# stgl/scarplet

Hardware: AMD Instinct MI355X
Metric: Mpixel·template/s (DEM pixels × ages × orientations / s) (higher is better)
Workload: dtype f32

## Files before the change

scarplet_amd/csrc/sc_fft.hip:

```cpp
#include "sc_internal.h"
#include <math.h>
#include <type_traits>
#include <string.h>

struct TileDev {
    int i0, j0, vy, vx, gi0, gj0;
};

#ifndef SC_I1_XLANE
#define SC_I1_XLANE 1
#endif
#ifndef SC_I2_RD1
#define SC_I2_RD1 1
#endif
#ifndef SC_LDS_WR1
#define SC_LDS_WR1 0
#endif
#ifndef SC_LDS_RD1
#define SC_LDS_RD1 1
#endif
#ifndef SC_H2_XLANE
#define SC_H2_XLANE 1
#endif
#ifndef SC_F1C_HOLD
// ... 593 lines not shown
                                              : make_float2(va[u], vb[u]);
        }
        lds_barrier();
        if (!SC_DBGBIT(dbg, 2)) fft4_lines<TX, false, true>(sm, twr);
#if SC_F1C_HOLD
        if (step + 1 < 2 * RBW && (!MIX || ((step + 1) & 1) == 0)) fetch(rb0 + ((step + 1) >> 1));
#else
        if (step + 1 < 2 * RBW) fetch(rb0 + ((step + 1) >> 1));
#endif
        float2* out = blk + (size_t)(pair * 2 + pl) * plane + (size_t)rb * 4 * TX;
        if (!SC_DBGBIT(dbg, 4))
#pragma unroll 4
        for (int e = 2 * tid; e < 4 * TX; e += 2 * NT) {
            int cb = e >> 4, rr = (e >> 2) & 3, cc = e & 3;
            float2 x0 = sm[lidx<TX>(rr, 4 * cb + cc)], x1 = sm[lidx<TX>(rr, 4 * cb + cc + 1)];
            *reinterpret_cast<float4*>(out + e) = make_float4(x0.x, x0.y, x1.x, x1.y);
        }
        lds_barrier();
    }
}

__global__ void __launch_bounds__(64)
k_tile_norms(const double* __restrict__ part, int nrb, double* __restrict__ norms) {
    const double2* p = reinterpret_cast<const double2*>(part) + (size_t)blockIdx.x * nrb;
    double s2 = 0.0, s4 = 0.0;
    for (int i = threadIdx.x; i < nrb; i += 64) {
        const double2 v = p[i];
        s2 += v.x;
        s4 += v.y;
    }
    for (int sft = 32; sft > 0; sft >>= 1) {
        s2 += __shfl_down(s2, sft, 64);
        s4 += __shfl_down(s4, sft, 64);
    }
    if (threadIdx.x == 0) {
        norms[2 * blockIdx.x] = s2;
        norms[2 * blockIdx.x + 1] = s4;
    }
}

__device__ __forceinline__ bool templ_rowblock_used(const TemplDev& t, int rb, int Ty) {
    bool any = false;
#pragma unroll
    for (int rr = 0; rr < 4; ++rr) {
        int r = 4 * rb + rr;
        int p = (r <= t.pmax) ? r : r - Ty;
        any |= p >= t.pmin && p <= t.pmax;
    }
    return any;
}

template <int TX>
__global__ void __launch_bounds__(fft_threads(TX), fft_waves(TX))
k_fwd_rows_templ(const TemplDev* __restrict__ templ, int first,
                 const float* __restrict__ win_w,
                 const uint8_t* __restrict__ win_m,
                 const double* __restrict__ sums, int Ty,
                 const float2* __restrict__ tw, float2* __restrict__ blk) {
    extern __shared__ __attribute__((aligned(16))) float2 sm[];
    FftTw<TX> twr;
    twr.load(tw);
    constexpr int NT = fft_threads(TX);
    const int rb = blockIdx.x;
    const TemplDev t = templ[first + blockIdx.y];
    const float alpha = sc_fft_alpha(sums, first + blockIdx.y);
    const size_t plane = (size_t)Ty * TX;
    float2* out = blk + (size_t)blockIdx.y * plane + (size_t)rb * 4 * TX;
    bool any = false;
    int prow[4];
#pragma unroll
    for (int rr = 0; rr < 4; ++rr) {
        int r = 4 * rb + rr;
        int p = (r <= t.pmax) ? r : r - Ty;
        prow[rr] = (p >= t.pmin && p <= t.pmax) ? p : INT_MIN;
        any |= prow[rr] != INT_MIN;
    }
    if (!any) return;
    {
        constexpr int NF = 4 * TX / NT;
        float w[NF];
        uint8_t m[NF];
#pragma unroll
        for (int u = 0; u < NF; ++u) {
            const int e = threadIdx.x + u * NT;
            const int rr = e / TX, s = e - rr * TX;
            const int q = (s <= t.qmax) ? s : s - TX;
            w[u] = 0.f;
            m[u] = 0;
            if (prow[rr] != INT_MIN && q >= t.qmin && q <= t.qmax) {
                size_t o = (size_t)t.win_off + (size_t)(prow[rr] - t.pmin) * t.ww + (q - t.qmin);
                w[u] = win_w[o];
                m[u] = win_m[o];
            }
        }
#pragma unroll
        for (int u = 0; u < NF; ++u) {
            const int e = threadIdx.x + u * NT;
            const int rr = e / TX, s = e - rr * TX;
            sm[lidx<TX>(rr, s)] = make_float2(alpha * w[u], m[u] ? 1.f : 0.f);
        }
    }
    lds_barrier();
    fft4_lines<TX, false>(sm, twr);
#pragma unroll 4
    for (int e = 2 * threadIdx.x; e < 4 * TX; e += 2 * NT) {
        int cb = e >> 4, rr = (e >> 2) & 3, cc = e & 3;
        float2 x0 = sm[lidx<TX>(rr, 4 * cb + cc)], x1 = sm[lidx<TX>(rr, 4 * cb + cc + 1)];
        *reinterpret_cast<float4*>(out + e) = make_float4(x0.x, x0.y, x1.x, x1.y);
    }
}

template <int TY>
__global__ void __launch_bounds__(fft_threads(TY), fft_waves(TY))
k_fwd_cols(const float2* __restrict__ blk, int Tx, const float2* __restrict__ tw,
           float2* __restrict__ out0, float2* __restrict__ out1, int split2,
           const TemplDev* __restrict__ templ) {
    extern __shared__ __attribute__((aligned(16))) float2 sm[];
    FftTw<TY> twr;
    twr.load(tw);
    constexpr int NT = fft_threads(TY);
    const int cb = blockIdx.x, q = blockIdx.y;
    const size_t plane = (size_t)TY * Tx;
    const float2* in = blk + (size_t)q * plane;
    const int nbx = Tx >> 2;
    TemplDev t{};
    if (templ) t = templ[q];
    constexpr int EP = (4 * TY + 2 * NT - 1) / (2 * NT);
    float4 x[EP];
#pragma unroll
    for (int u = 0; u < EP; ++u) {
        const int e = 2 * ((int)threadIdx.x + u * NT);
        x[u] = make_float4(0.f, 0.f, 0.f, 0.f);
        if (e < 4 * TY && (!templ || templ_rowblock_used(t, e >> 4, TY)))
            x[u] = *reinterpret_cast<const float4*>(in + ((size_t)(e >> 4) * nbx + cb) * 16 + (e & 15));
    }
#pragma unroll
    for (int u = 0; u < EP; ++u) {
        const int e = 2 * ((int)threadIdx.x + u * NT);
        if (e >= 4 * TY) continue;
        const int rbk = e >> 4, rr = (e >> 2) & 3, cc = e & 3;
        sm[lidx<TY>(cc, 4 * rbk + rr)] = make_float2(x[u].x, x[u].y);
        sm[lidx<TY>(cc + 1, 4 * rbk + rr)] = make_float2(x[u].z, x[u].w);
    }
    lds_barrier();
    fft4_lines<TY, false, true>(sm, twr);
    float2* out = split2 ? ((q & 1) ? out1 : out0) + (size_t)(q >> 1) * plane
                         : out0 + (size_t)q * plane;
    out += (size_t)cb * 4 * TY;
#pragma unroll 4
    for (int e = 2 * threadIdx.x; e < 4 * TY; e += 2 * NT) {
        int cc = e / TY, fy = e - cc * TY;
        float2 x0 = sm[lidx<TY>(cc, fy)], x1 = sm[lidx<TY>(cc, fy + 1)];
        *reinterpret_cast<float4*>(out + e) = make_float4(x0.x, x0.y, x1.x, x1.y);
    }
}

__host__ __device__ constexpr size_t half_plane(int Ty, int Tx) { return (size_t)(Tx / 2 + 4) * Ty; }

__global__ void __launch_bounds__(256)
k_split_templ(const float2* __restrict__ vh, int Ty, int Tx,
              float2* __restrict__ wh, float2* __restrict__ mh) {
    const size_t plane = (size_t)Ty * Tx, hplane = half_plane(Ty, Tx);
    const float2* v = vh + (size_t)blockIdx.y * plane;
    size_t e = ((size_t)blockIdx.x * 256 + threadIdx.x) * 2;
    if (e >= hplane) return;
    int fx = (int)(e / Ty), fy = (int)(e - (size_t)fx * Ty);
    const float2* vm = v + (size_t)((Tx - fx) & (Tx - 1)) * Ty;
    float4 a = *reinterpret_cast<const float4*>(v + e);
    float2 b0 = vm[(Ty - fy) & (Ty - 1)];
    float2 b1 = vm[Ty - fy - 1];
    float4 w = make_float4(0.5f * (a.x + b0.x), 0.5f * (a.y - b0.y),
                           0.5f * (a.z + b1.x), 0.5f * (a.w - b1.y));
    float4 m = make_float4(0.5f * (a.y + b0.y), -0.5f * (a.x - b0.x),
                           0.5f * (a.w + b1.y), -0.5f * (a.z - b1.x));
    *reinterpret_cast<float4*>(wh + (size_t)blockIdx.y * hplane + e) = w;
    *reinterpret_cast<float4*>(mh + (size_t)blockIdx.y * hplane + e) = m;
}

__device__ __forceinline__ float2 phase_tab(const float2* __restrict__ phy, const float2* __restrict__ phx,
                                            int fy, int fx) {
    const float2 a = phy[fy], b = phx[fx];
    return make_float2(a.x * b.x - a.y * b.y, a.x * b.y + a.y * b.x);
}
__global__ void __launch_bounds__(256)
k_split_templ_sym(const float2* __restrict__ vh, int Ty, int Tx, const float2* __restrict__ phy,
                  const float2* __restrict__ phx, int parity,
                  float* __restrict__ wa, float* __restrict__ mb) {
    const size_t plane = (size_t)Ty * Tx, hplane = half_plane(Ty, Tx);
    const float2* v = vh + (size_t)blockIdx.y * plane;
    size_t e = ((size_t)blockIdx.x * 256 + threadIdx.x) * 2;
    if (e >= hplane) return;
    int fx = (int)(e / Ty), fy = (int)(e - (size_t)fx * Ty);
    const float2* vm = v + (size_t)((Tx - fx) & (Tx - 1)) * Ty;
    float4 a = *reinterpret_cast<const float4*>(v + e);
    float2 b0 = vm[(Ty - fy) & (Ty - 1)];
    float2 b1 = vm[Ty - fy - 1];
    float2 w[2] = {make_float2(0.5f * (a.x + b0.x), 0.5f * (a.y - b0.y)),
                   make_float2(0.5f * (a.z + b1.x), 0.5f * (a.w - b1.y))};
    float2 m[2] = {make_float2(0.5f * (a.y + b0.y), -0.5f * (a.x - b0.x)),
                   make_float2(0.5f * (a.w + b1.y), -0.5f * (a.z - b1.x))};
    float ra[2], rb[2];
#pragma unroll
    for (int k = 0; k < 2; ++k) {
        float2 ph_ = phase_tab(phy, phx, fy + k, fx);
        float wr = w[k].x * ph_.x + w[k].y * ph_.y, wi = w[k].y * ph_.x - w[k].x * ph_.y;
        ra[k] = parity == 1 ? wi : wr;
        rb[k] = m[k].x * ph_.x + m[k].y * ph_.y;
    }
    *reinterpret_cast<float2*>(wa + (size_t)blockIdx.y * hplane + e) = make_float2(ra[0], ra[1]);
    *reinterpret_cast<float2*>(mb + (size_t)blockIdx.y * hplane + e) = make_float2(rb[0], rb[1]);
}

template <int TY>
__global__ void __launch_bounds__(fft_threads(TY), fft_waves(TY))
k_fwd_cols_tsym(const float2* __restrict__ blk, int Tx, const float2* __restrict__ tw,
                const TemplDev* __restrict__ templ, const float2* __restrict__ phx, int parity,
                float* __restrict__ wa, float* __restrict__ mb) {
    const float2* phy = tw + TY;
    extern __shared__ __attribute__((aligned(16))) float2 sm[];
    FftTw<TY> twr;
    twr.load(tw);
    constexpr int NT = fft_threads(TY);
    constexpr int EP = (4 * TY + 2 * NT - 1) / (2 * NT);
    const int cb = blockIdx.x, q = blockIdx.y;
    const size_t plane = (size_t)TY * Tx, hplane = half_plane(TY, Tx);
    const float2* in = blk + (size_t)q * plane;
    const int nbx = Tx >> 2;
    const TemplDev t = templ[q];
    float4 x[EP];
    {
        constexpr int NM = 4 * TY / NT;
        float2 v[NM];
#pragma unroll
        for (int u = 0; u < NM; ++u) {
            const int e = threadIdx.x + u * NT;
            const int c = e / TY, r = e - c * TY;
            const int col = (Tx - (4 * cb + c)) & (Tx - 1);
            v[u] = make_float2(0.f, 0.f);
            if (templ_rowblock_used(t, r >> 2, TY))
                v[u] = in[((size_t)(r >> 2) * nbx + (col >> 2)) * 16 + (r & 3) * 4 + (col & 3)];
        }
#pragma unroll
        for (int u = 0; u < NM; ++u) {
            const int e = threadIdx.x + u * NT;
            const int c = e / TY, r = e - c * TY;
            sm[lidx<TY>(c, r)] = v[u];
        }
#pragma unroll
        for (int u = 0; u < EP; ++u) {
            const int e = 2 * (threadIdx.x + u * NT);
            x[u] = make_float4(0.f, 0.f, 0.f, 0.f);
            if (e < 4 * TY && templ_rowblock_used(t, e >> 4, TY))
                x[u] = *reinterpret_cast<const float4*>(in + ((size_t)(e >> 4) * nbx + cb) * 16 + (e & 15));
        }
    }
    lds_barrier();
    fft4_lines<TY, false, true>(sm, twr);
    float2 vm0[EP], vm1[EP];
#pragma unroll
    for (int u = 0; u < EP; ++u) {
        const int e = 2 * (threadIdx.x + u * NT);
        if (e < 4 * TY) {
            const int cc = e / TY, fy = e - cc * TY;
            vm0[u] = sm[lidx<TY>(cc, (TY - fy) & (TY - 1))];
            vm1[u] = sm[lidx<TY>(cc, TY - fy - 1)];
        }
    }
    lds_barrier();
#pragma unroll
    for (int u = 0; u < EP; ++u) {
        const int e = 2 * (threadIdx.x + u * NT);
        if (e >= 4 * TY) continue;
        const int rbk = e >> 4, rr = (e >> 2) & 3, cc = e & 3;
        sm[lidx<TY>(cc, 4 * rbk + rr)] = make_float2(x[u].x, x[u].y);
        sm[lidx<TY>(cc + 1, 4 * rbk + rr)] = make_float2(x[u].z, x[u].w);
    }
    lds_barrier();
    fft4_lines<TY, false, true>(sm, twr);
#pragma unroll
    for (int u = 0; u < EP; ++u) {
        const int e = 2 * (threadIdx.x + u * NT);
        if (e >= 4 * TY) continue;
        const int cc = e / TY, fy = e - cc * TY, fx = 4 * cb + cc;
        const float2 a0 = sm[lidx<TY>(cc, fy)], a1 = sm[lidx<TY>(cc, fy + 1)];
        const float2 b0 = vm0[u], b1 = vm1[u];
        float2 w[2] = {make_float2(0.5f * (a0.x + b0.x), 0.5f * (a0.y - b0.y)),
                       make_float2(0.5f * (a1.x + b1.x), 0.5f * (a1.y - b1.y))};
        float2 m[2] = {make_float2(0.5f * (a0.y + b0.y), -0.5f * (a0.x - b0.x)),
                       make_float2(0.5f * (a1.y + b1.y), -0.5f * (a1.x - b1.x))};
        float ra[2], rb[2];
#pragma unroll
        for (int k = 0; k < 2; ++k) {
            float2 ph_ = phase_tab(phy, phx, fy + k, fx);
            float wr = w[k].x * ph_.x + w[k].y * ph_.y, wi = w[k].y * ph_.x - w[k].x * ph_.y;
            ra[k] = parity == 1 ? wi : wr;
            rb[k] = m[k].x * ph_.x + m[k].y * ph_.y;
        }
        const size_t o = (size_t)q * hplane + (size_t)cb * 4 * TY + e;
        *reinterpret_cast<float2*>(wa + o) = make_float2(ra[0], ra[1]);
        *reinterpret_cast<float2*>(mb + o) = make_float2(rb[0], rb[1]);
    }
}

template <int TY>
__host__ __device__ constexpr bool inv_cols_park() { return TY <= 2048; }
template <int TY>
// ... 160 lines not shown
        const float* hsrc = (pl ? mb : wa) + (size_t)vfirst * hplane +
                            (mirrored ? (size_t)(Tx - 4 * cb - 3) * TY : col);
        auto fetch = [&](int gi_) {
            const float* p = hsrc + (size_t)(PT ? 2 * gi_ : gi_) * hplane;
#pragma unroll
            for (int u = 0; u < EP; ++u)
                hreg[u] = *reinterpret_cast<const float2*>(p + 2 * (threadIdx.x + u * NT));
            if constexpr (PT) {
                const bool has2 = 2 * gi_ + 1 < G;
                const uint2* p2 = reinterpret_cast<const uint2*>(has2 ? p + hplane : p);
                const unsigned keep = has2 ? ~0u : 0u;
#pragma unroll
                for (int u = 0; u < EP; ++u) {
                    const uint2 r = p2[threadIdx.x + u * NT];
                    hreg2[u] = make_float2(__uint_as_float(r.x & keep), __uint_as_float(r.y & keep));
                }
            }
        };
        auto prod = [&](float2 x, float2 xb, float a, float a2) {
            if constexpr (XP) return make_float2(x.x * a - xb.y * a2, x.y * a + xb.x * a2);
            return PT ? make_float2(x.x * a - x.y * a2, x.x * a2 + x.y * a) : make_float2(a * x.x, a * x.y);
        };
        const float4* uuB = reinterpret_cast<const float4*>((pl ? uc2 : uc) + (size_t)pairB * plane + col);
        const bool rot = pl == 0 && parity == 1;
        float2 pvv[EP][2];
#pragma unroll
        for (int u = 0; u < EP; ++u) {
            const int e = 2 * (threadIdx.x + u * NT);
            const int cc = e / TY, fy = e - cc * TY, fx = 4 * cb + cc;
#pragma unroll
            for (int k = 0; k < 2; ++k) {
                if (!mirrored)
                    pvv[u][k] = phase_tab(tw + TY, phx, fy + k, fx);
                else {
                    pvv[u][k] = phase_tab(tw + TY, phx, (TY - fy - k) & (TY - 1), (Tx - fx) & (Tx - 1));
                    pvv[u][k].y = -pvv[u][k].y;
                }
            }
        }
        asm volatile("" ::: "memory");
        float4 xall[EP], xallB[XP ? EP : 1];
#pragma unroll
        for (int u = 0; u < EP; ++u) xall[u] = uu[threadIdx.x + u * NT];
        if constexpr (XP) {
#pragma unroll
            for (int u = 0; u < EP; ++u) xallB[u] = uuB[threadIdx.x + u * NT];
        }
        auto park = [&](const float4 x, const float2 (&pv)[2], float4* dst, int u) {
            float2 xv[2] = {make_float2(x.x, x.y), make_float2(x.z, x.w)};
#pragma unroll
            for (int k = 0; k < 2; ++k) {
                float2 v = cmul(xv[k], pv[k]);
                if (rot) v = mirrored ? make_float2(v.y, -v.x) : make_float2(-v.y, v.x);
                xv[k] = v;
            }
            dst[threadIdx.x + u * NT] = make_float4(xv[0].x, xv[0].y, xv[1].x, xv[1].y);
        };
#pragma unroll
        for (int u = 0; u < EP; ++u) park(xall[u], pvv[u], xs, u);
        if constexpr (XP) {
#pragma unroll
            for (int u = 0; u < EP; ++u) park(xallB[u], pvv[u], xsB, u);
        }
        if (SC_DBGBIT(dbg, 2) || (mirrored && SC_DBGBIT(dbg, 1))) {
#pragma unroll
            for (int u = 0; u < EP; ++u) hreg[u] = make_float2(1.f + u, 2.f);
        } else
        fetch(0);
        if (mirrored) lds_barrier();
        for (int gi_ = 0; gi_ < NG; ++gi_) {
            if (!mirrored) {
#pragma unroll
                for (int u = 0; u < EP; ++u) {
                    int e = 2 * (threadIdx.x + u * NT);
                    int cc = e / TY, fy = e - cc * TY;
                    const float4 x = xs[threadIdx.x + u * NT], xb = XP ? xsB[threadIdx.x + u * NT] : x;
                    sm[lidx<TY>(cc, fy)] = prod(make_float2(x.x, x.y), make_float2(xb.x, xb.y), hreg[u].x, hreg2[PT ? u : 0].x);
                    sm[lidx<TY>(cc, fy + 1)] = prod(make_float2(x.z, x.w), make_float2(xb.z, xb.w), hreg[u].y, hreg2[PT ? u : 0].y);
                }
            } else {
                const float2* x2 = reinterpret_cast<const float2*>(xs);
                const float2* x2B = reinterpret_cast<const float2*>(XP ? xsB : xs);
#pragma unroll
                for (int u = 0; u < EP; ++u) {
                    int e = 2 * (threadIdx.x + u * NT);
                    int sc = e / TY, m = e - sc * TY;
                    int cc = 3 - sc;
                    int f0 = (TY - m) & (TY - 1), f1 = (TY - m - 1) & (TY - 1);
                    float2 x0 = x2[cc * TY + f0], x1 = x2[cc * TY + f1];
                    sm[lidx<TY>(cc, f0)] = prod(x0, x2B[cc * TY + f0], hreg[u].x, hreg2[PT ? u : 0].x);
                    sm[lidx<TY>(cc, f1)] = prod(x1, x2B[cc * TY + f1], hreg[u].y, hreg2[PT ? u : 0].y);
                }
            }
            lds_barrier();
            if (gi_ + 1 < NG && !SC_DBGBIT(dbg, 2) && !(mirrored && SC_DBGBIT(dbg, 1))) fetch(gi_ + 1);
            if (!SC_DBGBIT(dbg, 8)) fft4_lines<TY, true>(sm, twr);
            float2* o = (pl ? ym : yw) + (size_t)gi_ * plane + (size_t)(cb >> 1) * 16 + (cb & 1) * 8;
            const int e_lo = 4 * rp_lo, e_hi = 4 * (rp_hi + 1);
            if (!SC_DBGBIT(dbg, 4))
#pragma unroll 2
            for (int e = e_lo + threadIdx.x; e < e_hi; e += NT) {
                int rp = e >> 2, k = e & 3;
                float2 x0 = sm[lidx<TY>(k, 2 * rp)], x1 = sm[lidx<TY>(k, 2 * rp + 1)];
#ifdef SC_ABLATE
                if (dbg & (16 | 32 | 64 | 128 | 256)) {
                    float2* dst = o + (size_t)rp * (Tx >> 3) * 16 + 2 * k;
                    if (dbg & 16)
                        dst = (pl ? ym : yw) + (size_t)gi_ * plane + (size_t)(cb >> 1) * 16 +
                              (size_t)((rp & ~1) + (cb & 1)) * (Tx >> 3) * 16 + (rp & 1) * 8 + 2 * k;
                    if (dbg & 128)
                        dst = (pl ? ym : yw) + (size_t)gi_ * plane + (size_t)cb * (TY * 4) + 2 * (size_t)e;
                    store_flavour(dst, x0, x1, (dbg & 32) ? 1 : (dbg & 64) ? 2 : (dbg & 256) ? 3 : 0);
                    continue;
                }
#endif
                store_stream(o + (size_t)rp * (Tx >> 3) * 16 + 2 * k, x0, x1);
            }
            lds_barrier();
        }
    }
}


template <int TY, bool MIRROR, bool PT>
__global__ void __launch_bounds__(fft_threads(TY), 2)
k_inv_cols_sym(const float2* __restrict__ uc, const float2* __restrict__ uc2,
               const float* __restrict__ wa, const float* __restrict__ mb, int Tx,
               int cb0, int pair, int vfirst, int G, int rp_lo, int rp_hi, const float2* __restrict__ phx,
               int parity, const float2* __restrict__ tw, float2* __restrict__ yw,
               float2* __restrict__ ym, int ystride, int dbg, int np, int pcj, int tstride,
               const TileDev* __restrict__ tiles, int py_valid) {
    inv_cols_sym_body<TY, MIRROR, PT>((int)blockIdx.x, uc, uc2, wa, mb, Tx, cb0, pair, vfirst, G, rp_lo, rp_hi, phx,
                                      parity, tw, yw, ym, ystride, dbg, np, pcj, tstride, tiles, py_valid);
}

template <int TY, bool PT, bool XP = false>
__global__ void __launch_bounds__(fft_threads(TY), 2)
k_inv_cols_symx(const float2* __restrict__ uc, const float2* __restrict__ uc2,
                const float* __restrict__ wa, const float* __restrict__ mb, int Tx,
                int pair, int vfirst, int G, int rp_lo, int rp_hi, const float2* __restrict__ phx,
                int parity, const float2* __restrict__ tw, float2* __restrict__ yw,
                float2* __restrict__ ym, int ystride, int dbg, int np, int pcj, int tstride,
                const TileDev* __restrict__ tiles, int py_valid) {
    const int j = blockIdx.x, i = ((j >> 4) << 3) | (j & 7);
    if constexpr (!XP) TAKE_TEMPLATE_SHARE(PT, (size_t)TY * Tx)
    if ((j >> 3) & 1)
        inv_cols_sym_body<TY, true, PT, XP>((Tx >> 2) - 1 - i, uc, uc2, wa, mb, Tx, 0, pair, vfirst, G, rp_lo, rp_hi, phx,
                                            parity, tw, yw, ym, ystride, dbg, np, pcj, tstride, tiles, py_valid);
    else
        inv_cols_sym_body<TY, false, PT, XP>(i, uc, uc2, wa, mb, Tx, 0, pair, vfirst, G, rp_lo, rp_hi, phx,
                                             parity, tw, yw, ym, ystride, dbg, np, pcj, tstride, tiles, py_valid);
}

template <int TY>
__host__ __device__ constexpr int w8_line() { return TY + TY / 16 + 4; }
template <int TY>
__host__ __device__ constexpr size_t w8_lds() {
    return ((size_t)8 * w8_line<TY>() + (SC_I1_TWTAB ? 16 : 4) * (TY / 16 + TY / 256) + SC_MAX_GROUP) * sizeof(float2);
}

template <int TY, bool MIRROR, bool PT, int NC>
__device__ __forceinline__ void
inv_cols_w8_body(const int B, const int jobx, const float2* __restrict__ uc, const float2* __restrict__ uc2,
                 const float* __restrict__ wa, const float* __restrict__ mb, int Tx,
                 int pair, int vfirst, int G, int rp_lo, int rp_hi, const float2* __restrict__ phx,
                 int parity, const float2* __restrict__ tw, float2* __restrict__ yw,
                 float2* __restrict__ ym, int ystride, int np, int pcj, int tstride,
                 const TileDev* __restrict__ tiles, int py_valid, const TemplDev* __restrict__ tl) {
    extern __shared__ __attribute__((aligned(16))) float2 sm[];
    constexpr int S = TY / 16;
    static_assert(S % 64 == 0 && S / 64 <= 2, "one wave per line: 64 or 128 sets");
    constexpr int U = S / 64;
    constexpr int NK = 16 * U;
    constexpr int LINE = w8_line<TY>();
    const int w = __builtin_amdgcn_readfirstlane(threadIdx.x >> 6), lane = threadIdx.x & 63;
    float2* line = sm + w * LINE;
    int i0A = 0, i0B = 0, vyA = 0, vyB = 0;
    {
        const int ob = jobx / pcj, q = jobx - ob * pcj;
        const TileDev tA_ = tiles[2 * (pair + q)], tB_ = tiles[2 * (pair + q) + 1];
        i0A = tA_.i0; i0B = tB_.i0; vyA = tA_.vy; vyB = tB_.vy;
        if (py_valid >= 0) {
            const int vy = max(tA_.vy, tB_.vy);
            rp_hi = min(rp_hi, (py_valid + vy - 1) >> 1);
        }
        pair += ob * np + q;
        vfirst += ob * tstride;
    }
    int2* const rng = reinterpret_cast<int2*>(sm + NC * LINE + (SC_I1_TWTAB ? 16 : 4) * (S + S / 16));
    {
        const int NGt = PT ? (G + 1) / 2 : G;
        const int gi_ = threadIdx.x;
        if (gi_ < NGt) {
            int lo = rp_lo, hi = rp_hi;
            if (tl && py_valid >= 0) {
                int klo = INT_MAX, khi = INT_MIN;
#pragma unroll
                for (int k = 0; k < (PT ? 2 : 1); ++k) {
                    const int ti = vfirst + (PT ? 2 * gi_ + k : gi_);
                    if (PT && k == 1 && 2 * gi_ + 1 >= G) break;
                    const int ilo = tl[ti].ilo, ihi = tl[ti].ihi;
                    if (vyA > 0) { klo = min(klo, ilo - i0A); khi = max(khi, ihi - i0A); }
                    if (vyB > 0) { klo = min(klo, ilo - i0B); khi = max(khi, ihi - i0B); }
                }
                if (khi < klo) { lo = 1; hi = 0; }
                else {
                    lo = max(lo, (max(klo, 0) + py_valid) >> 1);
                    hi = min(hi, (min(khi, TY) + py_valid) >> 1);
                }
            }
            rng[gi_] = make_int2(lo, hi);
        }
    }
    const size_t plane = (size_t)TY * Tx, hplane = half_plane(TY, Tx);
    yw += (size_t)jobx * ystride * plane;
    ym += (size_t)jobx * ystride * plane;
    const int ft = NC * B + w;
    const int fs = MIRROR ? Tx - ft : ft;
    float2* t1 = sm + NC * LINE;
#if SC_I1_TWTAB
    float2* t2 = t1 + 16 * S;
    for (int i = threadIdx.x; i < S + S / 16; i += 64 * NC) {
        const bool st2 = i >= S;
        const int e = st2 ? (i - S) << 4 : i, n = st2 ? S / 16 : S;
        float2* t = st2 ? t2 + (i - S) : t1 + i;
        const float2 wb[4] = {tw[e], tw[2 * e], tw[4 * e], tw[8 * e]};
        pk::v2 wk[16];
        twiddle16_expand(wb, wk);
#pragma unroll
        for (int k = 1; k < 16; ++k) t[k * n] = make_float2(wk[k].x, wk[k].y);
    }
#else
    float2* t2 = t1 + 4 * S;
    for (int i = threadIdx.x; i < 4 * S; i += 64 * NC) t1[i] = tw[(i % S) << (i / S)];
    for (int i = threadIdx.x; i < 4 * (S / 16); i += 64 * NC) t2[i] = tw[((i % (S / 16)) << 4) << (i / (S / 16))];
#endif
    auto tw_of = [&](const float2* t, int n, int idx, float2 (&wq)[4]) {
#pragma unroll
        for (int m = 0; m < 4; ++m) wq[m] = lds_cell<true>(t + m * n + idx);
    };
    float c[NK], c2[PT ? NK : 1];
    const int NG = PT ? (G + 1) / 2 : G;
    for (int pl = 0; pl < 2; ++pl) {
        const float2* xcol = (pl ? uc2 : uc) + (size_t)pair * plane + (size_t)ft * TY;
        const float* hsrc = (pl ? mb : wa) + (size_t)vfirst * hplane + (size_t)fs * TY;
        const bool rot = pl == 0 && parity == 1;
        float2 xp[NK];
#pragma unroll
        for (int k = 0; k < NK; ++k) {
            const int fy = lane + 64 * k;
            float2 pv;
            if (!MIRROR) {
                pv = phase_tab(tw + TY, phx, fy, ft);
            } else {
                pv = phase_tab(tw + TY, phx, (TY - fy) & (TY - 1), (Tx - ft) & (Tx - 1));
                pv.y = -pv.y;
            }
            float2 v = cmul(xcol[fy], pv);
            if (rot) v = MIRROR ? make_float2(v.y, -v.x) : make_float2(-v.y, v.x);
            xp[k] = v;
        }
        const float* cbase = hsrc + (MIRROR ? TY - lane : lane);
        const int c0off = (MIRROR && lane == 0) ? -TY : 0;
        auto fetch = [&](int gi_, int u) {
            const float* p = cbase + (size_t)(PT ? 2 * gi_ : gi_) * hplane;
            const bool has2 = PT && 2 * gi_ + 1 < G;
            const float* p2 = has2 ? p + hplane : p;
            const unsigned keep2 = has2 ? ~0u : 0u;
#pragma unroll
            for (int k = 0; k < NK; ++k) {
                if (u >= 0 && k % U != u) continue;
                const int off = k ? (MIRROR ? -64 * k : 64 * k) : c0off;
                c[k] = p[off];
                if constexpr (PT) c2[k] = __uint_as_float(__float_as_uint(p2[off]) & keep2);
            }
        };
        fetch(0, -1);
        for (int gi_ = 0; gi_ < NG; ++gi_) {
            lds_barrier();
            float2 wq[4];
            int lt = lane;
            asm volatile("" : "+v"(lt));
#pragma unroll
            for (int u = 0; u < U; ++u) {
                float2 a1[16];
#pragma unroll
                for (int j = 0; j < 16; ++j) {
                    const int k = u + U * j;
                    a1[j] = PT ? make_float2(xp[k].x * c[k] - xp[k].y * c2[k], xp[k].x * c2[k] + xp[k].y * c[k])
                               : make_float2(c[k] * xp[k].x, c[k] * xp[k].y);
                }
#if SC_I1_TWTAB
                set_compute_store<TY, 16, 0, true, true>(line, lt + 64 * u, a1, wq, t1 + lt + 64 * u, S);
#else
                tw_of(t1, S, lt + 64 * u, wq);
                set_compute_store<TY, 16, 0, true, false, true>(line, lt + 64 * u, a1, wq);
#endif
            }
            constexpr bool SPLIT = PT && U > 1 && NC == 8;
            if (gi_ + 1 < NG) fetch(gi_ + 1, SPLIT ? 0 : -1);
            asm volatile("" ::: "memory");
            float2 a[U][16];
#pragma unroll
            for (int u = 0; u < U; ++u) set_load<TY, true>(line, lt + 64 * u, a[u]);
            constexpr bool XLANE = SC_I1_XLANE && (TY == 2048 || TY == 1024);
            if constexpr (XLANE) {
                float2 o2[U][16];
#pragma unroll
// ... 1152 lines not shown
        h[T + k] = make_float2((float)cos(b), (float)sin(b));
    }
    int rc = sc_ensure(ctx, buf, sizeof(float2) * h.size());
    if (rc) return rc;
    SC_HIP(ctx, hipStreamSynchronize(ctx->stream));
    SC_HIP(ctx, hipMemcpy(buf.p, h.data(), sizeof(float2) * h.size(), hipMemcpyHostToDevice));
    have = key;
    return SC_OK;
}

static int npairs_of(const FftGeom& fg) { return (fg.ntiles + 1) / 2; }

void fft_spectra_forget(sc_ctx* ctx) {
    std::fill(ctx->spec_key.begin(), ctx->spec_key.end(), NAN);
}

int fft_prepare(sc_ctx* ctx, const FftGeom& fg, int n_templ_chunk, int group, int nb, int n_slots) {
    if (!fft_size_supported(fg.Ty) || !fft_size_supported(fg.Tx))
        return sc_fail(ctx, SC_ERR_UNSUPPORTED, "FFT tile %dx%d not supported", fg.Ty, fg.Tx);
    int rc;
    if ((rc = upload_twiddles(ctx, ctx->tw_y, ctx->tw_Ty, fg.Ty, 1 - ctx->g.oy))) return rc;
    if ((rc = upload_twiddles(ctx, ctx->tw_x, ctx->tw_Tx, fg.Tx, 1 - ctx->g.ox))) return rc;
    const Geom& g = ctx->g;
    int np = npairs_of(fg);
    std::vector<TileDev> h(2 * np);
    for (int k = 0; k < 2 * np; ++k) {
        TileDev t{0, 0, 0, 0, 0, 0};
        if (k < fg.ntiles) {
            int ty = k / fg.ntx, tx = k % fg.ntx;
            t.i0 = g.cy0 + ty * fg.Vy;
            t.j0 = g.cx0 + tx * fg.Vx;
            t.vy = std::min(fg.Vy, g.cy1 - t.i0);
            t.vx = std::min(fg.Vx, g.cx1 - t.j0);
            t.gi0 = t.i0 + g.oy - fg.Py;
            t.gj0 = t.j0 + g.ox - fg.Qx;
        }
        h[k] = t;
    }
    {
        const size_t bytes = sizeof(TileDev) * h.size();
        const void* before = ctx->tiles.p;
        if ((rc = sc_ensure(ctx, ctx->tiles, bytes))) return rc;
        if (before != ctx->tiles.p || ctx->h_tiles.size() != bytes || memcmp(ctx->h_tiles.data(), h.data(), bytes) != 0) {
            SC_HIP(ctx, hipStreamSynchronize(ctx->stream));
            ctx->h_tiles.assign((const unsigned char*)h.data(), (const unsigned char*)h.data() + bytes);
            SC_HIP(ctx, hipMemcpyAsync(ctx->tiles.p, ctx->h_tiles.data(), bytes, hipMemcpyHostToDevice, ctx->stream));
        }
    }
    size_t plane = (size_t)fg.Ty * fg.Tx * sizeof(float2);
    size_t nblk = std::max((size_t)2 * np * nb, (size_t)n_templ_chunk);
    if ((rc = sc_ensure(ctx, ctx->blk, plane * nblk))) return rc;
    {
        const Geom& gg = ctx->g;
        const long long sig[24] = {fg.Ty, fg.Tx, fg.Vy, fg.Vx, fg.nty, fg.ntx, fg.circ_y, fg.circ_x, fg.Py, fg.Qx,
                                   gg.ly, gg.lx, gg.gy0, gg.gx0, gg.ny, gg.nx, gg.cy0, gg.cy1, gg.cx0, gg.cx1,
                                   gg.wrap, n_slots, 0, 0};
        bool keep = n_slots > 0 && 2.0 * (double)plane * np * n_slots <= ctx->spec_mb * 1048576.0;
        if (keep) {
            const double add = 2.0 * (double)plane * np * n_slots - (double)(ctx->uc.cap + ctx->uc2.cap);
            size_t free_b = 0, total_b = 0;
            if (add > 0.0 && (hipMemGetInfo(&free_b, &total_b) != hipSuccess || add > 0.25 * (double)free_b))
                keep = false;
        }
        const int slots = keep ? n_slots : 0;
        const size_t have = std::max(nb, slots);
        if (ctx->uc.cap > 2 * plane * np * have + ((size_t)256 << 20)) {
            SC_HIP(ctx, hipStreamSynchronize(ctx->stream));
            for (DevBuf* b : {&ctx->uc, &ctx->uc2}) {
                if (b->p) SC_HIP(ctx, hipFree(b->p));
                b->p = nullptr;
                b->cap = 0;
            }
        }
        const void *p0 = ctx->uc.p, *p1 = ctx->uc2.p, *p2 = ctx->norms.p;
        if ((rc = sc_ensure(ctx, ctx->norms, sizeof(double) * 2 * np * have))) return rc;
        if ((rc = sc_ensure(ctx, ctx->uc, plane * np * have))) return rc;
        if ((rc = sc_ensure(ctx, ctx->uc2, plane * np * have))) return rc;
        if (!keep || slots != ctx->spec_slots || memcmp(sig, ctx->spec_sig, sizeof(sig)) != 0 ||
            p0 != ctx->uc.p || p1 != ctx->uc2.p || p2 != ctx->norms.p) {
            ctx->spec_key.assign((size_t)3 * slots, NAN);
            memcpy(ctx->spec_sig, sig, sizeof(sig));
        }
        ctx->spec_slots = slots;
        ctx->spec_uc_stride = (size_t)np * fg.Ty * fg.Tx;
        ctx->spec_norm_stride = (size_t)2 * np;
        ctx->uc_off = ctx->norms_off = 0;
    }
    if ((rc = sc_ensure(ctx, ctx->norm_part, sizeof(double) * 2 * np * nb * (fg.Ty / 4)))) return rc;
    if ((rc = sc_ensure(ctx, ctx->curv, sizeof(float) * (size_t)ctx->g.ly * ctx->g.lx * nb))) return rc;
    if ((rc = sc_ensure(ctx, ctx->vh, plane * n_templ_chunk))) return rc;
    size_t hplane = half_plane(fg.Ty, fg.Tx) * sizeof(float2);
    if ((rc = sc_ensure(ctx, ctx->wh, hplane * n_templ_chunk))) return rc;
    if ((rc = sc_ensure(ctx, ctx->mh, hplane * n_templ_chunk))) return rc;
    int pb = 1;
    {
        size_t free_b = 0, total_b = 0;
        double budget = 0.0;
        if (hipMemGetInfo(&free_b, &total_b) == hipSuccess)
            budget = std::min(32e9, 0.25 * (double)(free_b + ctx->yw.cap + ctx->ym.cap));
        if (ctx->y_gb > 0.0) budget = ctx->y_gb * 1e9;
        double per_pair = 2.0 * (double)plane * group * nb;
        pb = (int)std::max(1.0, std::min((double)np, floor(budget / per_pair)));
    }
    ctx->fft_pb = pb;
    if ((rc = sc_ensure(ctx, ctx->yw, plane * group * pb * nb))) return rc;
    if ((rc = sc_ensure(ctx, ctx->ym, plane * group * pb * nb))) return rc;
    return SC_OK;
}

int fft_batch_orientations(const sc_ctx* ctx, const FftGeom& fg, int n_per, int group) {
    if (ctx->batch_off || n_per < 1 || n_per > group) return 1;
    const bool fast = (fg.Tx == 512 || fg.Tx == 1024 || fg.Tx == 2048) && ctx->variant != 9;
    if (!fast) return 1;
    const int np = (fg.ntiles + 1) / 2;
    const int cap = ctx->batch_templ > 0 ? ctx->batch_templ : SC_MAX_BATCH;
    const int by_table = (SC_MAX_GROUP / n_per >= 3 || cap <= SC_MAX_GROUP) ? std::min(cap, SC_MAX_GROUP) / n_per : cap / n_per;
    const int by_fill = (ctx->batch_fill > 0 ? ctx->batch_fill : 4096) / std::max(1, np * (fg.Tx / 8));
    return std::max(1, std::min(std::min(by_table, by_fill), SC_MAX_ORIENT));
}

static int sib_slots(sc_ctx* ctx, size_t n, SibSync& out) {
    const size_t bytes = n * sizeof(uint32_t);
    if (bytes > ctx->sib_buf.cap || ctx->sib_epoch >= 0xFFFFFEu) {
        int rc = sc_ensure(ctx, ctx->sib_buf, std::max(bytes, (size_t)1 << 20));
        if (rc) return rc;
        SC_HIP(ctx, hipMemsetAsync(ctx->sib_buf.p, 0, ctx->sib_buf.cap, ctx->stream));
        ctx->sib_epoch = 0;
    }
    out.slots = (uint32_t*)ctx->sib_buf.p;
    out.base = (++ctx->sib_epoch) << 8;
    return SC_OK;
}

template <typename K>
static int set_lds(sc_ctx* ctx, K kernel, size_t bytes) {
    return sc_lds_attr(ctx, (const void*)kernel, bytes);
}

#define DISPATCH_T(T, FN)                                                     \
    switch (T) {                                                              \
        case 64: FN(64); break;                                               \
        case 128: FN(128); break;                                             \
        case 256: FN(256); break;                                             \
        case 512: FN(512); break;                                             \
        case 1024: FN(1024); break;                                           \
        case 2048: FN(2048); break;                                           \
        case 4096: FN(4096); break;                                           \
        default: return sc_fail(ctx, SC_ERR_UNSUPPORTED, "tile size %d", T);  \
    }

static int launch_fwd_cols(sc_ctx* ctx, const FftGeom& fg, int nplanes,
                           float2* out0, float2* out1, int split2,
                           const TemplDev* templ = nullptr) {
    size_t lds = fft_lds_bytes(fg.Ty);
    dim3 grid(fg.Tx / 4, nplanes);
    sc_prof_begin(ctx, SC_K_FWD_COLS);
#define FN(T)                                                                  \
    {                                                                          \
        int rc = set_lds(ctx, k_fwd_cols<T>, lds);                             \
        if (rc) return rc;                                                     \
        hipLaunchKernelGGL(k_fwd_cols<T>, grid, dim3(fft_threads(T)), lds,     \
                           ctx->stream, (const float2*)ctx->blk.p, fg.Tx,      \
                           (const float2*)ctx->tw_y.p, out0, out1, split2,     \
                           templ);                                             \
    }
    DISPATCH_T(fg.Ty, FN)
#undef FN
    sc_prof_end(ctx);
    SC_HIP(ctx, hipGetLastError());
    return SC_OK;
}

int fft_forward_curv(sc_ctx* ctx, const FftGeom& fg, int nb, const float (*coef)[3]) {
    int np = npairs_of(fg);
    size_t lds = fft_lds_bytes(fg.Tx);
    dim3 grid(fg.Ty / 4 / FWD_ROWS_RBW, np * nb);
    CurvMix mixc;
    memset(&mixc, 0, sizeof(mixc));
    if (coef) {
        if (nb > SC_MAX_ORIENT) return sc_fail(ctx, SC_ERR_INVALID, "curvature batch of %d planes", nb);
        for (int b = 0; b < nb; ++b)
            for (int j = 0; j < 3; ++j) mixc.c[b][j] = coef[b][j];
    }
    sc_prof_begin(ctx, SC_K_FWD_ROWS);
#define FN2(T, MIXV)                                                           \
    {                                                                          \
        int rc = set_lds(ctx, k_fwd_rows_curv<T, MIXV>, lds);                  \
        if (rc) return rc;                                                     \
        hipLaunchKernelGGL((k_fwd_rows_curv<T, MIXV>), grid, dim3(fft_threads(T)), \
                           lds, ctx->stream, (const float*)(MIXV ? ctx->A.p : ctx->curv.p), \
                           (const float*)ctx->B.p, (const float*)ctx->C.p, mixc, \
                           ctx->g, (const TileDev*)ctx->tiles.p, fg.Ty,        \
                           (const float2*)ctx->tw_x.p, (float2*)ctx->blk.p,    \
                           (double*)ctx->norm_part.p, ctx->dbg, np,            \
                           (size_t)ctx->g.ly * ctx->g.lx);                     \
    }
#define FN(T) { if (coef) FN2(T, true) else FN2(T, false) }
    DISPATCH_T(fg.Tx, FN)
#undef FN
#undef FN2
    hipLaunchKernelGGL(k_tile_norms, dim3(np * nb), dim3(64), 0, ctx->stream,
                       (const double*)ctx->norm_part.p, fg.Ty / 4, (double*)ctx->norms.p + ctx->norms_off);
    sc_prof_end(ctx);
    SC_HIP(ctx, hipGetLastError());
    return launch_fwd_cols(ctx, fg, 2 * np * nb, (float2*)ctx->uc.p + ctx->uc_off, (float2*)ctx->uc2.p + ctx->uc_off, 1);
}

static bool fft_use_sym(const sc_ctx* ctx, const FftGeom& fg, int parity) {
    return parity != 0 && fg.Ty <= 2048 && ctx->variant != 8;
}

int fft_forward_templates(sc_ctx* ctx, const FftGeom& fg, int first, int n, int parity) {
    size_t lds = fft_lds_bytes(fg.Tx);
    dim3 grid(fg.Ty / 4, n);
    sc_prof_begin(ctx, SC_K_FWD_ROWS);
#define FN(T)                                                                  \
    {                                                                          \
        int rc = set_lds(ctx, k_fwd_rows_templ<T>, lds);                       \
        if (rc) return rc;                                                     \
        hipLaunchKernelGGL(k_fwd_rows_templ<T>, grid, dim3(fft_threads(T)),    \
                           lds, ctx->stream, (const TemplDev*)ctx->templ.p,    \
                           first, (const float*)ctx->win_w.p,                  \
                           (const uint8_t*)ctx->win_m.p,                       \
                           (const double*)ctx->sums.p, fg.Ty,                  \
                           (const float2*)ctx->tw_x.p, (float2*)ctx->blk.p);   \
    }
    DISPATCH_T(fg.Tx, FN)
#undef FN
    sc_prof_end(ctx);
    SC_HIP(ctx, hipGetLastError());
    if (fft_use_sym(ctx, fg, parity) && ctx->variant != 7) {
        size_t ldsc = fft_lds_bytes(fg.Ty);
        dim3 gridc(fg.Tx / 8 + 1, n);
        sc_prof_begin(ctx, SC_K_FWD_COLS);
#define FN(T)                                                                  \
    {                                                                          \
        int rc = set_lds(ctx, k_fwd_cols_tsym<T>, ldsc);                       \
        if (rc) return rc;                                                     \
        hipLaunchKernelGGL(k_fwd_cols_tsym<T>, gridc, dim3(fft_threads(T)), ldsc, ctx->stream, \
                           (const float2*)ctx->blk.p, fg.Tx, (const float2*)ctx->tw_y.p, \
                           (const TemplDev*)ctx->templ.p + first, (const float2*)ctx->tw_x.p + fg.Tx, \
                           parity, (float*)ctx->wh.p, (float*)ctx->mh.p);      \
    }
        switch (fg.Ty) {
            case 64: FN(64); break;
            case 128: FN(128); break;
            case 256: FN(256); break;
            case 512: FN(512); break;
            case 1024: FN(1024); break;
            default: FN(2048); break;
        }
#undef FN
        sc_prof_end(ctx);
        SC_HIP(ctx, hipGetLastError());
        return SC_OK;
    }
    int rc = launch_fwd_cols(ctx, fg, n, (float2*)ctx->vh.p, nullptr, 0,
                             (const TemplDev*)ctx->templ.p + first);
    if (rc) return rc;
    size_t cells = half_plane(fg.Ty, fg.Tx);
    dim3 grid_s((unsigned)((cells / 2 + 255) / 256), n);
    sc_prof_begin(ctx, SC_K_FWD_COLS);
    if (fft_use_sym(ctx, fg, parity))
        hipLaunchKernelGGL(k_split_templ_sym, grid_s, dim3(256), 0, ctx->stream,
                           (const float2*)ctx->vh.p, fg.Ty, fg.Tx, (const float2*)ctx->tw_y.p + fg.Ty,
                           (const float2*)ctx->tw_x.p + fg.Tx,
                           parity, (float*)ctx->wh.p, (float*)ctx->mh.p);
    else
        hipLaunchKernelGGL(k_split_templ, grid_s, dim3(256), 0, ctx->stream, (const float2*)ctx->vh.p,
                           fg.Ty, fg.Tx, (float2*)ctx->wh.p, (float2*)ctx->mh.p);
    sc_prof_end(ctx);
    SC_HIP(ctx, hipGetLastError());
    return SC_OK;
}

int fft_inverse_fold(sc_ctx* ctx, const FftGeom& fg, int first, int n,
                     int group, bool to_maps, bool full_masks, int parity, int nb) {
    const bool sym = fft_use_sym(ctx, fg, parity);
    int np = npairs_of(fg);
    size_t lds_r = fft_lds_bytes(fg.Tx);
    int rp_lo = 0, rp_hi = fg.Ty / 2 - 1;
    if (!fg.circ_y) {
        rp_lo = fg.Py / 2;
        rp_hi = std::min(fg.Ty - 1, fg.Py + fg.Vy - 1) / 2;
    }
    const int rp_n = rp_hi - rp_lo + 1;
    if (group > SC_MAX_GROUP)
        return sc_fail(ctx, SC_ERR_INVALID, "group %d exceeds %d", group, SC_MAX_GROUP);
    const int pb = std::max(1, ctx->fft_pb);
    const size_t yblock = (size_t)fg.Ty * fg.Tx * group;
    const bool fast = (fg.Tx == 512 || fg.Tx == 1024 || fg.Tx == 2048) && ctx->variant != 9;
    const bool symx = sym && ctx->variant != 6 && fg.Ty >= 512 && fg.Ty <= 2048 && (fg.Tx / 8) % 8 == 0;
    const bool w8 = symx && ctx->variant != 2 && (fg.Ty == 2048 || fg.Ty == 1024) && (fg.Tx / 16) % 8 == 0;
    if (nb > 1 && (!fast || n > group || nb * n > SC_MAX_BATCH || n > SC_MAX_GROUP))
        return sc_fail(ctx, SC_ERR_INVALID, "orientation batching outside its conditions");
    auto chunk = [&](int pair0, int pc, auto ptc) -> int {
        constexpr bool PTV = decltype(ptc)::value;
        for (int g0 = 0; g0 < n; g0 += group) {
            int G = std::min(group, n - g0);
            const bool xp = PTV && n == 1 && nb >= 2 && pc == 1 && sym && symx && fg.Ty == 512 &&
                            ctx->variant != 12 && !to_maps;
            const size_t lds_c = (size_t)4 * fft_line(fg.Ty) * sizeof(float2) +
                                 (fg.Ty <= 2048 ? (size_t)4 * fg.Ty * sizeof(float2) : 0);
            const int slots = 256 * (int)std::max<size_t>(1, (size_t)(160 * 1024) / lds_c);
            int pi1 = nb > 1 ? pc : std::max(1, std::min(pc, (slots + fg.Tx / 8 - 1) / (fg.Tx / 8)));
            int jil = 1;
            if (nb == 1 && w8 && (!PTV || fg.Ty == 1024) && ctx->variant != 1 && !xp && ctx->i1_pairs > 1) {
                jil = std::min(pc, ctx->i1_pairs);
                pi1 = jil;
// ... 312 lines not shown
```

Before: 191,600.

## Add wave-per-line forward column FFT kernel for 1024/2048 tiles

Adds a new forward column FFT kernel in which each of 8 waves owns one column line in LDS. It processes several column groups per block, prefetching the next group's global loads into registers while computing the current one. The later radix stages run in registers with cross-lane transposes, and results are written straight to global memory. It replaces the generic k_fwd_cols for Ty of 1024 or 2048 unless variant 21 is selected, trading more register pressure and code complexity for fewer LDS round-trips and barriers.

```diff
diff --git a/scarplet_amd/csrc/sc_fft.hip b/scarplet_amd/csrc/sc_fft.hip
--- a/scarplet_amd/csrc/sc_fft.hip
+++ b/scarplet_amd/csrc/sc_fft.hip
@@ -769,6 +769,140 @@
         int cc = e / TY, fy = e - cc * TY;
         float2 x0 = sm[lidx<TY>(cc, fy)], x1 = sm[lidx<TY>(cc, fy + 1)];
         *reinterpret_cast<float4*>(out + e) = make_float4(x0.x, x0.y, x1.x, x1.y);
+    }
+}
+
+template <int TY>
+__host__ __device__ constexpr int w8_line() { return TY + TY / 16 + 4; }
+constexpr int FWD_W8_CPW = 4;
+template <int TY>
+__host__ __device__ constexpr size_t fwd_w8_lds() {
+    return ((size_t)8 * w8_line<TY>() + 4 * (TY / 16 + TY / 256)) * sizeof(float2);
+}
+template <int TY, bool TEMPL>
+__global__ void __launch_bounds__(512, TY == 1024 ? 4 : 2)
+k_fwd_cols_w8(const float2* __restrict__ blk, int Tx, const float2* __restrict__ tw,
+              float2* __restrict__ out0, float2* __restrict__ out1, int split2,
+              const TemplDev* __restrict__ templ) {
+    extern __shared__ __attribute__((aligned(16))) float2 sm[];
+    constexpr int S = TY / 16;
+    static_assert(S % 64 == 0 && S / 64 <= 2, "one wave per line: 64 or 128 sets");
+    constexpr int U = S / 64;
+    constexpr int LINE = w8_line<TY>();
+    const int w = __builtin_amdgcn_readfirstlane(threadIdx.x >> 6), lane = threadIdx.x & 63;
+    float2* line = sm + w * LINE;
+    const int q = blockIdx.y;
+    const size_t plane = (size_t)TY * Tx;
+    const float2* in = blk + (size_t)q * plane;
+    const int nbx = Tx >> 2;
+    float2* out = split2 ? ((q & 1) ? out1 : out0) + (size_t)(q >> 1) * plane : out0 + (size_t)q * plane;
+    TemplDev t{};
+    if constexpr (TEMPL) t = templ[q];
+    float2* t1 = sm + 8 * LINE;
+    float2* t2 = t1 + 4 * S;
+    for (int i = threadIdx.x; i < 4 * S; i += 512) t1[i] = tw[(i % S) << (i / S)];
+    for (int i = threadIdx.x; i < 4 * (S / 16); i += 512) t2[i] = tw[((i % (S / 16)) << 4) << (i / (S / 16))];
+    auto tw_of = [&](const float2* t, int n, int idx, float2 (&wq)[4]) {
+#pragma unroll
+        for (int m = 0; m < 4; ++m) wq[m] = lds_cell<true>(t + m * n + idx);
+    };
+    const int g0 = blockIdx.x * FWD_W8_CPW;
+    const int ng = min(FWD_W8_CPW, (Tx >> 3) - g0);
+    constexpr int NP = TY / 128;
+    float4 x[NP];
+    auto fetch = [&](int g, bool real) {
+#pragma unroll
+        for (int i = 0; i < NP; ++i) {
+            const int e = (int)threadIdx.x + 512 * i, rb = e >> 4;
+            const float2* src = in + (real ? ((size_t)rb * nbx + 2 * g) * 16 + 2 * (e & 15) : 0);
+            if constexpr (TEMPL) {
+                x[i] = make_float4(0.f, 0.f, 0.f, 0.f);
+                if (templ_rowblock_used(t, rb, TY)) x[i] = *reinterpret_cast<const float4*>(src);
+            } else {
+                x[i] = *reinterpret_cast<const float4*>(src);
+            }
+        }
+    };
+    auto fill = [&]() {
+#pragma unroll
+        for (int i = 0; i < NP; ++i) {
+            const int e = (int)threadIdx.x + 512 * i;
+            const int r = 4 * (e >> 4) + ((e & 7) >> 1), l = 4 * ((e >> 3) & 1) + 2 * (e & 1);
+            sm[l * LINE + ph(r)] = make_float2(x[i].x, x[i].y);
+            sm[(l + 1) * LINE + ph(r)] = make_float2(x[i].z, x[i].w);
+        }
+    };
+    auto stage1 = [&]() {
+        int lt = lane;
+        asm volatile("" : "+v"(lt));
+        float2 wq[4];
+        float2 a[U][16];
+#pragma unroll
+        for (int u = 0; u < U; ++u) set_load<TY, true>(line, lt + 64 * u, a[u]);
+        asm volatile("" ::: "memory");
+#pragma unroll
+        for (int u = 0; u < U; ++u) {
+            tw_of(t1, S, lt + 64 * u, wq);
+            set_compute_store<TY, 16, 0, false, false, true>(line, lt + 64 * u, a[u], wq);
+        }
+        asm volatile("" ::: "memory");
+    };
+    auto stage23 = [&](int fx) {
+        int lt = lane;
+        asm volatile("" : "+v"(lt));
+        float2 wq[4];
+        float2 a[U][16];
+#pragma unroll
+        for (int u = 0; u < U; ++u) set_load<TY, true>(line, lt + 64 * u, a[u]);
+        float2 o2[U][16];
+#pragma unroll
+        for (int u = 0; u < U; ++u) {
+            tw_of(t2, S / 16, (lt + 64 * u) >> 4, wq);
+            set_compute_regs<false>(a[u], wq, o2[u]);
+        }
+        asm volatile("" ::: "memory");
+#pragma unroll
+        for (int u = 0; u < U; ++u)
+#pragma unroll
+            for (int mh = 0; mh < 4; ++mh) {
+                xlane_transpose4(o2[u][4 * mh].x, o2[u][4 * mh + 1].x, o2[u][4 * mh + 2].x, o2[u][4 * mh + 3].x);
+                xlane_transpose4(o2[u][4 * mh].y, o2[u][4 * mh + 1].y, o2[u][4 * mh + 2].y, o2[u][4 * mh + 3].y);
+            }
+        constexpr int R3 = TY / 256, NB3 = 16 / R3;
+        float2* ocol = out + (size_t)fx * TY + lt;
+#pragma unroll
+        for (int u3 = 0; u3 < U; ++u3)
+#pragma unroll
+            for (int b = 0; b < NB3; ++b) {
+                pk::v2 v[R3];
+#pragma unroll
+                for (int j = 0; j < R3; ++j) {
+                    const float2 x = o2[j >> 2][4 * (u3 + U * b) + (j & 3)];
+                    v[j] = pk::v2{x.x, x.y};
+                }
+                pk::B<R3, false>::run(v);
+#pragma unroll
+                for (int m = 0; m < R3; ++m) {
+                    const pk::v2 y = v[pk::B<R3, false>::pos(m)];
+                    ocol[64 * u3 + S * b + 256 * m] = make_float2(y.x, y.y);
+                }
+            }
+    };
+    const int fx0 = 8 * g0 + w;
+    fetch(g0, true);
+    lds_barrier();
+    fill();
+    fetch(ng > 1 ? g0 + 1 : g0, ng > 1);
+    lds_barrier();
+    for (int gi = 0;; ++gi) {
+        stage1();
+        stage23(fx0 + 8 * gi);
+        if (gi + 1 >= ng) break;
+        lds_barrier();
+        fill();
+        asm volatile("" ::: "memory");
+        fetch(gi + 2 < ng ? g0 + gi + 2 : g0, gi + 2 < ng);
+        lds_barrier();
     }
 }
 
@@ -1235,8 +1369,6 @@
                                              parity, tw, yw, ym, ystride, dbg, np, pcj, tstride, tiles, py_valid);
 }
 
-template <int TY>
-__host__ __device__ constexpr int w8_line() { return TY + TY / 16 + 4; }
 template <int TY>
 __host__ __device__ constexpr size_t w8_lds() {
     return ((size_t)8 * w8_line<TY>() + (SC_I1_TWTAB ? 16 : 4) * (TY / 16 + TY / 256) + SC_MAX_GROUP) * sizeof(float2);
@@ -2695,9 +2827,28 @@
 static int launch_fwd_cols(sc_ctx* ctx, const FftGeom& fg, int nplanes,
                            float2* out0, float2* out1, int split2,
                            const TemplDev* templ = nullptr) {
+    sc_prof_begin(ctx, SC_K_FWD_COLS);
+    if ((fg.Ty == 2048 || fg.Ty == 1024) && ctx->variant != 21) {
+        dim3 gridw((fg.Tx / 8 + FWD_W8_CPW - 1) / FWD_W8_CPW, nplanes);
+#define FN2(T, TM)                                                             \
+    {                                                                          \
+        int rc = set_lds(ctx, k_fwd_cols_w8<T, TM>, fwd_w8_lds<T>());          \
+        if (rc) return rc;                                                     \
+        hipLaunchKernelGGL((k_fwd_cols_w8<T, TM>), gridw, dim3(512), fwd_w8_lds<T>(), \
+                           ctx->stream, (const float2*)ctx->blk.p, fg.Tx,      \
+                           (const float2*)ctx->tw_y.p, out0, out1, split2,     \
+                           templ);                                             \
+    }
+#define FN(T) { if (templ) FN2(T, true) else FN2(T, false) }
+        if (fg.Ty == 2048) FN(2048) else FN(1024)
+#undef FN2
+#undef FN
+        sc_prof_end(ctx);
+        SC_HIP(ctx, hipGetLastError());
+        return SC_OK;
+    }
     size_t lds = fft_lds_bytes(fg.Ty);
     dim3 grid(fg.Tx / 4, nplanes);
-    sc_prof_begin(ctx, SC_K_FWD_COLS);
 #define FN(T)                                                                  \
     {                                                                          \
         int rc = set_lds(ctx, k_fwd_cols<T>, lds);                             \
```

After: 192,000, median of 6. About the same (+0.2%).
